# j4n1k/rl4co-slap

Measured on AMD Instinct MI355X. Metric: env-steps/sec (batch×decode) SLAP & TSP-100 at 1/2/4/8 MI355X, higher is better.
Workload: dtype u8+i64+f32

## Files before the change

rl4co_slap_amd/csrc/nearest.hip:

```cpp
#include "co_common.hpp"

using namespace co;

namespace {

constexpr int kNoNode = 0x7fffffff;

#ifndef CO_NEAREST_LDS_G
#define CO_NEAREST_LDS_G 4
#endif
#ifndef CO_NEAREST_CVRP_G
#define CO_NEAREST_CVRP_G 8
#endif

__global__ __launch_bounds__(256) void cvrp_pad_kernel(int64_t B, const int32_t* __restrict__ len,
                                                       const int32_t* __restrict__ tmax,
                                                       int64_t* __restrict__ acts_out,
                                                       int64_t* __restrict__ cur_out,
                                                       float* __restrict__ used_out) {
  const int T = *tmax;
  for (int64_t b = (int64_t)blockIdx.x * blockDim.x + threadIdx.x; b < B;
       b += (int64_t)gridDim.x * blockDim.x) {
    const int L = len[b];
    for (int t = L; t < T; ++t) acts_out[(int64_t)t * B + b] = 0;
    if (L < T) {
      cur_out[b] = 0;
      used_out[b] = 0.f;
    }
  }
}

typedef float v2f __attribute__((ext_vector_type(2)));

constexpr int clog2(int v) {
  int b = 0;
  while ((1 << b) < v) ++b;
  return b;
}

__device__ __forceinline__ uint32_t med3u(uint32_t a, uint32_t b, uint32_t c) {
  uint32_t r;
  asm("v_med3_u32 %0, %1, %2, %3" : "=v"(r) : "v"(a), "v"(b), "v"(c));
  return r;
}

template <int G, int EPL>
__device__ __forceinline__ void lds_load_x(const float* __restrict__ rowx, int sl,
                                           v2f (&x2)[EPL / 2]) {
  const float* r = rowx + sl;
#pragma unroll
  for (int p = 0; p < EPL / 2; ++p) x2[p] = (v2f){r[2 * p * G], r[(2 * p + 1) * G]};
}

template <int G, int EPL, bool DEM>
__device__ __forceinline__ void lds_scan(const v2f (&x2)[EPL / 2], float cx, float cy,
                                         const v2f (&y2)[EPL / 2], const v2f (&dm2)[EPL / 2],
                                         float used, float vcap, uint32_t& m1, uint32_t& m2) {
  constexpr uint32_t BM = (1u << clog2(G * EPL)) - 1u;
  const v2f cx2 = {cx, cx}, cy2 = {cy, cy};
  const v2f u2 = {used, used};
  uint32_t a1 = 0xffffffffu, a2 = 0xffffffffu, b1 = 0xffffffffu, b2 = 0xffffffffu;
#pragma unroll
  for (int p = 0; p < EPL / 2; ++p) {
    const v2f dx = x2[p] - cx2, dy = y2[p] - cy2;
    const v2f s = dx * dx + dy * dy;
    v2f du = {0.f, 0.f};
    if (DEM) du = dm2[p] + u2;
#pragma unroll
    for (int h = 0; h < 2; ++h) {
      uint32_t key = (__float_as_uint(s[h]) & ~BM) | (uint32_t)((2 * p + h) * G);
      if (DEM && du[h] > vcap) key = 0xffffffffu;
      if (p & 1) {
        b2 = med3u(b1, b2, key);
        b1 = min(b1, key);
      } else {
        a2 = med3u(a1, a2, key);
        a1 = min(a1, key);
      }
    }
  }
  m1 = min(a1, b1);
  m2 = med3u(a1, b1, min(a2, b2));
}

template <int G>
__device__ __forceinline__ void grp_min2(uint32_t& m1, uint32_t& m2) {
#define CO_MIN2(C)                                             \
  {                                                            \
    const uint32_t t1 = dpp_u<C>(m1), t2 = dpp_u<C>(m2);       \
    m2 = med3u(m1, t1, min(m2, t2));                           \
    m1 = min(m1, t1);                                          \
  }
  if (G >= 2) CO_MIN2(0xB1);
  if (G >= 4) CO_MIN2(0x4E);
  if (G >= 8) CO_MIN2(0x141);
  if (G >= 16) CO_MIN2(0x140);
#undef CO_MIN2
  if (G >= 32) {
    const auto a = __builtin_amdgcn_permlane16_swap(m1, m1, false, false);
    const auto b = __builtin_amdgcn_permlane16_swap(m2, m2, false, false);
    m2 = med3u(a[0], a[1], min(b[0], b[1]));
    m1 = min(a[0], a[1]);
  }
  if (G >= 64) {
    const auto a = __builtin_amdgcn_permlane32_swap(m1, m1, false, false);
    const auto b = __builtin_amdgcn_permlane32_swap(m2, m2, false, false);
    m2 = med3u(a[0], a[1], min(b[0], b[1]));
    m1 = min(a[0], a[1]);
  }
}

template <int G, int EPL, bool DEM>
__device__ __noinline__ int lds_exact(const float* __restrict__ rowx,
                                      const float2* __restrict__ lrow,
                                      const float* __restrict__ drow, int lo, int hi, int sl,
                                      float cx, float cy, float used, float vcap) {
  float best = __builtin_inff();
  int bi = kNoNode;
#pragma unroll 2
  for (int k = 0; k < EPL; ++k) {
    const int c = k * G + sl;
    const int ci = c < lo ? 0 : (c > hi ? hi - lo : c - lo);
    const float d = edge_len(cx, cy, rowx[c], lrow[ci].y);
    const bool fits = !DEM || !(drow[ci] + used > vcap);
    if (fits && d < best) {
      best = d;
      bi = c;
    }
  }
  grp_argmin_split<G>(best, bi);
  return bi;
}

template <int G, int EPL, bool DEM>
__device__ __forceinline__ int lds_nearest(const float* __restrict__ rowx,
                                           const v2f (&x2)[EPL / 2], int sl, float cx, float cy,
                                           const v2f (&y2)[EPL / 2], const v2f (&dm2)[EPL / 2],
                                           float used, float vcap,
                                           const float2* __restrict__ lrow,
                                           const float* __restrict__ drow, int lo, int hi) {
  constexpr uint32_t BM = (1u << clog2(G * EPL)) - 1u;
  constexpr float kWin = 1.0f + (float)(1u << clog2(G * EPL)) * 0x1p-20f;
  uint32_t m1, m2;
  lds_scan<G, EPL, DEM>(x2, cx, cy, y2, dm2, used, vcap, m1, m2);
  m1 |= (uint32_t)sl;
  m2 |= (uint32_t)sl;
  grp_min2<G>(m1, m2);
  const uint32_t t1 = m1 & ~BM, t2 = m2 & ~BM;
  const bool none = t1 >= 0x7fc00000u;
  const bool ok = none | ((t1 - 0x0d800000u < 0x7f800000u - 0x0d800000u) &
                          (t2 > __float_as_uint(__uint_as_float(t1) * kWin)));
  int w = none ? kNoNode : (int)(m1 & BM);
  if (__builtin_expect(__any(!ok), 0))
    w = lds_exact<G, EPL, DEM>(rowx, lrow, drow, lo, hi, sl, cx, cy, used, vcap);
  return w;
}

template <int G>
struct TermAcc {
  double sum = 0.0;
  float hold = 0.f;
  __device__ __forceinline__ void add(float sq, int t, int sl) {
    const int r = t & (G - 1);
    hold = sl == r ? sq : hold;
    if (r == G - 1) {
      asm volatile("");
      sum += (double)__builtin_sqrtf(hold);
      hold = 0.f;
    }
  }
  __device__ __forceinline__ double total() {
    return grp_sum_f64<G>(sum + (double)__builtin_sqrtf(hold));
  }
};

template <int G, int EPL>
__global__ __launch_bounds__(64) void tsp_nearest_lds_kernel(
    int64_t B, int N, const float2* __restrict__ locs, int64_t* __restrict__ acts_out,
    uint8_t* __restrict__ mask_out, int64_t* __restrict__ first_out,
    int64_t* __restrict__ cur_out, int64_t* __restrict__ i_out, uint8_t* __restrict__ done_out,
    uint8_t* __restrict__ step_reward_out, float* __restrict__ reward_out) {
  static_assert(EPL % 2 == 0 && (G & (G - 1)) == 0 && G * EPL <= 1024, "slot pairs");
  constexpr int IPW = 64 / G, SLOTS = G * EPL;
  __shared__ float2 s_x[IPW * SLOTS / 2];
  const int lane = threadIdx.x, sl = lane % G, gi = lane / G, gbase = lane - sl;
  const int64_t base = (int64_t)blockIdx.x * IPW;
  if (base >= B) return;
  const int64_t b = base + gi;
  const bool valid = b < B;
  const int64_t bb = valid ? b : B - 1;
  const float2* lrow = locs + bb * N;
  float* const rowx = reinterpret_cast<float*>(s_x) + gi * SLOTS;
  const float qnan = __builtin_nanf("");
  v2f y2[EPL / 2];
#pragma unroll
  for (int k = 0; k < EPL; ++k) {
    const int c = k * G + sl;
    const float2 q = lrow[c < N ? c : N - 1];
    rowx[c] = c < N ? q.x : qnan;
    y2[k >> 1][k & 1] = c < N ? q.y : 0.f;
  }
  const v2f nodem[EPL / 2] = {};
  const float2 q0 = lrow[0];
  __syncthreads();
  rowx[0] = qnan;
  float cx = q0.x, cy = q0.y;
  if (valid && sl == 0) acts_out[bb] = 0;
  TermAcc<G> len;
  int cur = 0;
  v2f x2[EPL / 2];
  lds_load_x<G, EPL>(rowx, sl, x2);
  for (int t = 1; t < N; ++t) {
    int a = lds_nearest<G, EPL, false>(rowx, x2, sl, cx, cy, y2, nodem, 0.f, 0.f, lrow,
                                       nullptr, 0, N - 1);
    a = a == kNoNode ? 0 : a;
    float* px = rowx + a;
    const float2 wq = lrow[a];
    const float wx = wq.x, wy = wq.y;
    *px = qnan;
    lds_load_x<G, EPL>(rowx, sl, x2);
    const float dx = wx - cx, dy = wy - cy;
    len.add(dx * dx + dy * dy, t, sl);
    cx = wx;
    cy = wy;
    cur = a;
    if (valid && sl == 0) acts_out[(int64_t)t * B + bb] = a;
  }
  const float ex = q0.x - cx, ey = q0.y - cy;
  len.add(ex * ex + ey * ey, N, sl);
  const double tour = len.total();
  if (!valid) return;
  uint8_t* mrow = mask_out + bb * N;
  for (int c = sl; c < N; c += G) mrow[c] = 0;
  if (sl == 0) {
    first_out[bb] = 0;
    cur_out[bb] = cur;
    i_out[bb] = N;
    done_out[bb] = 1;
    step_reward_out[bb] = 0;
    reward_out[bb] = -(float)tour;
  }
}

template <int G, int EPL>
__global__ __launch_bounds__(64) void cvrp_nearest_lds_kernel(
    int64_t B, int N, const float2* __restrict__ depot, const float2* __restrict__ locs_in,
    const float* __restrict__ demand, float vcap, int max_steps, int64_t* __restrict__ acts_out,
    float2* __restrict__ locs_out, int64_t* __restrict__ cur_out, float* __restrict__ used_out,
    float* __restrict__ vcap_out, uint8_t* __restrict__ visited_out,
    uint8_t* __restrict__ mask_out, uint8_t* __restrict__ done_out,
    uint8_t* __restrict__ step_reward_out, float* __restrict__ reward_out,
    int32_t* __restrict__ len_out, int32_t* __restrict__ tmax, int32_t* status) {
  static_assert(EPL % 2 == 0 && (G & (G - 1)) == 0 && G * EPL <= 1024, "slot pairs");
  constexpr int IPW = 64 / G, SLOTS = G * EPL;
  __shared__ float2 s_x[IPW * SLOTS / 2];
  const int lane = threadIdx.x, sl = lane % G, gi = lane / G, gbase = lane - sl;
  const int M = N + 1;
  const int64_t base = (int64_t)blockIdx.x * IPW;
  if (base >= B) return;
  const int64_t b = base + gi;
  const bool valid = b < B;
  const int64_t bb = valid ? b : B - 1;
  const float2* lrow = locs_in + bb * N;
  const float* drow = demand + bb * N;
  float* const rowx = reinterpret_cast<float*>(s_x) + gi * SLOTS;
  const float qnan = __builtin_nanf("");
  const float2 dep = depot[bb];
  v2f y2[EPL / 2], dm2[EPL / 2];
#pragma unroll
  for (int k = 0; k < EPL; ++k) {
    const int c = k * G + sl;
    const int ci = c < 1 ? 0 : (c <= N ? c - 1 : N - 1);
    const float2 lq = lrow[ci];
    const float ld = drow[ci];
    const float2 q = c == 0 ? dep : (c <= N ? lq : make_float2(qnan, 0.f));
    const float d = (c >= 1 && c <= N) ? ld : 0.f;
    if (valid && locs_out && c <= N) locs_out[bb * M + c] = q;
    rowx[c] = c == 0 ? qnan : q.x;
    y2[k >> 1][k & 1] = q.y;
    dm2[k >> 1][k & 1] = d;
  }
  __syncthreads();
  float cx = dep.x, cy = dep.y, used = 0.f;
  uint32_t st = 0;
  int cur = 0;
  bool done = false;
  TermAcc<G> dist;
  v2f x2[EPL / 2];
  lds_load_x<G, EPL>(rowx, sl, x2);
  int t = 0;
  for (; t < max_steps; ++t) {
    if (__ballot(!done) == 0) break;
    const int w = lds_nearest<G, EPL, true>(rowx, x2, sl, cx, cy, y2, dm2, used, vcap, lrow,
                                            drow, 1, N);
    const int a = w == kNoNode ? 0 : w;
    float* px = rowx + a;
    const int ai = a == 0 ? 0 : a - 1;
    const float2 wq = lrow[ai];
    const float wx = wq.x, wy = wq.y, wd = drow[ai];
    if (!done && a != 0) *px = qnan;
    lds_load_x<G, EPL>(rowx, sl, x2);
    const float2 q = a == 0 ? dep : make_float2(wx, wy);
    const float dx = q.x - cx, dy = q.y - cy;
    dist.add(done ? 0.f : dx * dx + dy * dy, t, sl);
    if (done) continue;
    used = a != 0 ? (used + wd) * 1.0f : 0.0f;
    st = ((st & 0x8000ffffu) + (a != 0 ? 1u : 0u)) | ((uint32_t)(t + 1) << 16) |
         (a == 0 ? 0x80000000u : 0u);
    cur = a;
    cx = q.x;
    cy = q.y;
    if (valid && sl == 0) acts_out[(int64_t)t * B + bb] = a;
    done = (st & 0x8000ffffu) == (0x80000000u | (uint32_t)N);
  }
  const int len = (int)((st >> 16) & 0x7fffu);
  const float ex = dep.x - cx, ey = dep.y - cy;
  dist.add(ex * ex + ey * ey, t, sl);
  const double tour = dist.total();
  bool any_feas = false;
  uint8_t* vrow = visited_out + bb * M;
  uint8_t* mrow = mask_out + bb * M;
#pragma unroll
  for (int k = 0; k < EPL; ++k) {
    const int c = k * G + sl;
    const bool v = c == 0 ? (st >> 31) != 0 : __builtin_isnan(rowx[c]);
    const bool feas = c >= 1 && c <= N && !v && !(dm2[k >> 1][k & 1] + used > vcap);
    any_feas |= feas;
    if (valid && c <= N) {
      vrow[c] = v;
      if (c >= 1) mrow[c] = feas;
    }
  }
  const uint64_t gmask = (G == 64 ? ~0ull : ((1ull << G) - 1ull)) << gbase;
  const bool anyf = (__ballot(any_feas) & gmask) != 0;
  if (valid && sl == 0) {
    mrow[0] = !((cur == 0) && anyf);
    cur_out[bb] = cur;
    used_out[bb] = used;
    vcap_out[bb] = vcap;
    done_out[bb] = done;
    step_reward_out[bb] = 0;
    reward_out[bb] = -(float)tour;
    len_out[bb] = len;
    if (!done) set_status(status, CO_ST_TRUNCATED);
    atomicMax(tmax, len);
  }
}

inline unsigned lds_grid(int64_t B, int G) {
  return cover_grid(B, 64 / G, 64);
}

}

int co_internal_tsp_nearest_rollout(int64_t B, int64_t N, const float* locs, int64_t* acts_out,
                                    uint8_t* mask_out, int64_t* first_out, int64_t* cur_out,
                                    int64_t* i_out, uint8_t* done_out, uint8_t* step_reward_out,
                                    float* reward_out, void* stream) {
  const float2* l2 = reinterpret_cast<const float2*>(locs);
  hipStream_t s = (hipStream_t)stream;
  if (lds_grid(B, 4) == 0) return CO_E_INVAL;
#define CO_TSPL(G, EPL)                                                                        \
  hipLaunchKernelGGL((tsp_nearest_lds_kernel<G, EPL>), dim3(lds_grid(B, G)), dim3(64), 0, s, B,  \
                     (int)N, l2, acts_out, mask_out, first_out, cur_out, i_out, done_out,        \
                     step_reward_out, reward_out)
  if (N <= 32) CO_TSPL(4, 8);
  else if (N <= 64) CO_TSPL(4, 16);
  else if (N <= 104 && CO_NEAREST_LDS_G == 4) CO_TSPL(4, 26);
  else if (N <= 112) CO_TSPL(8, 14);
  else if (N <= 128) CO_TSPL(8, 16);
  else if (N <= 256) CO_TSPL(8, 32);
  else if (N <= 512) CO_TSPL(16, 32);
  else CO_TSPL(32, 32);
#undef CO_TSPL
  return launch_status();
}

extern "C" int co_cvrp_rollout(int64_t B, int64_t N, const float* depot, const float* locs,
                               const float* demand, float vcap, int64_t max_steps,
                               int64_t* acts_out, float* locs_out, int64_t* cur_out,
                               float* used_out, float* vcap_out, uint8_t* visited_out,
                               uint8_t* mask_out, uint8_t* done_out, uint8_t* step_reward_out,
                               float* reward_out, int32_t* len_out, int32_t* steps_out,
                               int32_t* status, void* stream) {
  if (B < 0 || B > 0x7fffffff || N <= 0 || N > 1023 || max_steps <= 0 || max_steps > 0x7fff)
    return CO_E_INVAL;
  if (B == 0) return CO_OK;
  if (!depot || !locs || !demand || !acts_out || !cur_out || !used_out || !vcap_out ||
      !visited_out || !mask_out || !done_out || !step_reward_out || !reward_out || !len_out ||
      !steps_out || !status)
    return CO_E_INVAL;
  if ((reinterpret_cast<uintptr_t>(depot) | reinterpret_cast<uintptr_t>(locs) |
       reinterpret_cast<uintptr_t>(locs_out)) & 7)
    return CO_E_ALIGN;
  hipStream_t s = (hipStream_t)stream;
  if (lds_grid(B, 4) == 0) return CO_E_INVAL;
  if (zero_i32(steps_out, s) != hipSuccess) return launch_status();
  const float2* d2 = reinterpret_cast<const float2*>(depot);
  const float2* l2 = reinterpret_cast<const float2*>(locs);
  float2* lo = reinterpret_cast<float2*>(locs_out);
  const int64_t M = N + 1;
#define CO_CVRPL(G, EPL)                                                                       \
  hipLaunchKernelGGL((cvrp_nearest_lds_kernel<G, EPL>), dim3(lds_grid(B, G)), dim3(64), 0, s, B, \
                     (int)N, d2, l2, demand, vcap, (int)max_steps, acts_out, lo, cur_out,        \
                     used_out, vcap_out, visited_out, mask_out, done_out, step_reward_out,       \
                     reward_out, len_out, steps_out, status)
  if (M <= 32) CO_CVRPL(4, 8);
  else if (M <= 64) CO_CVRPL(4, 16);
  else if (M <= 112) CO_CVRPL(CO_NEAREST_CVRP_G, 112 / CO_NEAREST_CVRP_G);
  else if (M <= 128) CO_CVRPL(8, 16);
  else if (M <= 256) CO_CVRPL(8, 32);
  else if (M <= 512) CO_CVRPL(16, 32);
  else CO_CVRPL(32, 32);
#undef CO_CVRPL
  hipLaunchKernelGGL(cvrp_pad_kernel, dim3(grid_for(B, 256, 2048)), dim3(256), 0, s, B, len_out,
                     steps_out, acts_out, cur_out, used_out);
  return launch_status();
}
```

Measured before the change: 353.9 billion.

## Compact unvisited TSP nodes into shrinking LDS slots during greedy decode

Restructures the greedy nearest-neighbour TSP decode into phases. As nodes are visited, the remaining live nodes are compacted into fewer per-lane slots with an index table stored in LDS, so each step's scan covers only the remaining candidates instead of all N. A packed min2 key with a tolerance window selects the winner, falling back to an exact scan when the gap between the two best candidates is ambiguous. It also raises the launch-bounds occupancy hint. The cost is added compaction passes with barriers, extra code paths and register pressure.

```diff
diff --git a/rl4co_slap_amd/csrc/nearest.hip b/rl4co_slap_amd/csrc/nearest.hip
--- a/rl4co_slap_amd/csrc/nearest.hip
+++ b/rl4co_slap_amd/csrc/nearest.hip
@@ -174,14 +174,168 @@
   }
 };
 
+constexpr int even_up(int v) { return (v + 1) & ~1; }
+
+constexpr int tsp_next_epl(int epl0, int idx_bytes, int epl) {
+  if (epl <= 2) return 0;
+  int n = even_up(epl >= 12 ? (2 * epl + 2) / 3 : (epl + 1) / 2);
+  const int room = (epl0 * 4 / (4 + idx_bytes)) & ~1;
+  if (epl == epl0 && n > room) n = room;
+  return n;
+}
+
+template <int G, class IdxT>
+__device__ __noinline__ int tsp_exact(const float* __restrict__ rowx, const IdxT* tab,
+                                      const float2* __restrict__ lrow, int N, int epl, int sl,
+                                      float cx, float cy) {
+  float best = __builtin_inff();
+  int bi = kNoNode;
+#pragma unroll 2
+  for (int k = 0; k < epl; ++k) {
+    const int p = k * G + sl;
+    int c = tab ? (int)tab[p] : p;
+    c = c < N ? c : N - 1;
+    const float d = edge_len(cx, cy, rowx[p], lrow[c].y);
+    if (d < best) {
+      best = d;
+      bi = p;
+    }
+  }
+  grp_argmin_split<G>(best, bi);
+  return bi;
+}
+
+template <int G, class IdxT>
+struct TspRun {
+  int64_t B, bb;
+  int N, sl, gbase, t, cur;
+  bool valid;
+  const float2* __restrict__ lrow;
+  float* rowx;
+  IdxT* tab;
+  int64_t* __restrict__ acts_out;
+  float cx, cy;
+  TermAcc<G> len;
+};
+
+template <int G, bool TAB, class IdxT>
+__device__ __forceinline__ void tsp_visit(TspRun<G, IdxT>& r, int w) {
+  const bool hit = w != kNoNode;
+  const int p = hit ? w : 0;
+  int a = p;
+  if (TAB) {
+    const int c = (int)r.tab[p];
+    a = hit ? c : 0;
+  }
+  const float2 wq = r.lrow[a];
+  const float wx = wq.x, wy = wq.y;
+  if (!TAB || hit) r.rowx[p] = __builtin_nanf("");
+  const float dx = wx - r.cx, dy = wy - r.cy;
+  r.len.add(dx * dx + dy * dy, r.t, r.sl);
+  r.cx = wx;
+  r.cy = wy;
+  r.cur = a;
+  if (r.valid && r.sl == 0) r.acts_out[(int64_t)r.t * r.B + r.bb] = a;
+}
+
+template <int G, int EPL, bool TAB, class IdxT>
+__device__ __forceinline__ void tsp_step(TspRun<G, IdxT>& r, v2f (&x2)[EPL / 2],
+                                         const v2f (&y2)[EPL / 2]) {
+  constexpr uint32_t BM = (1u << clog2(G * EPL)) - 1u;
+  constexpr float kWin = 1.0f + (float)(1u << clog2(G * EPL)) * 0x1p-20f;
+  const v2f nodem[EPL / 2] = {};
+  uint32_t m1, m2;
+  lds_scan<G, EPL, false>(x2, r.cx, r.cy, y2, nodem, 0.f, 0.f, m1, m2);
+  m1 |= (uint32_t)r.sl;
+  m2 |= (uint32_t)r.sl;
+  grp_min2<G>(m1, m2);
+  const uint32_t t1 = m1 & ~BM, t2 = m2 & ~BM;
+  const bool none = t1 >= 0x7fc00000u;
+  const bool ok = none | ((t1 - 0x0d800000u < 0x7f800000u - 0x0d800000u) &
+                          (t2 > __float_as_uint(__uint_as_float(t1) * kWin)));
+  int w = none ? kNoNode : (int)(m1 & BM);
+  if (__builtin_expect(__any(!ok), 0))
+    w = tsp_exact<G, IdxT>(r.rowx, TAB ? r.tab : nullptr, r.lrow, r.N, EPL, r.sl, r.cx, r.cy);
+  tsp_visit<G, TAB, IdxT>(r, w);
+  lds_load_x<G, EPL>(r.rowx, r.sl, x2);
+}
+
+template <int G, int EPL, int NEXT, bool TAB, class IdxT>
+__device__ __forceinline__ bool tsp_compact(const TspRun<G, IdxT>& r, const v2f (&x2)[EPL / 2],
+                                            v2f (&nx2)[NEXT / 2], v2f (&ny2)[NEXT / 2]) {
+  static_assert(G <= 32, "a group's ballot bits fit 32 bits");
+  const uint32_t gm = G == 32 ? 0xffffffffu : (1u << G) - 1u, lm = (1u << r.sl) - 1u;
+  uint32_t live = 0;
+#pragma unroll
+  for (int k = 0; k < EPL; ++k) live += x2[k >> 1][k & 1] == x2[k >> 1][k & 1] ? 1u : 0u;
+  live = grp_reduce<G>(live, [](uint32_t a, uint32_t b) { return a + b; });
+  if (__any(live > (uint32_t)(G * NEXT))) return false;
+  int node[TAB ? EPL : 1];
+  if (TAB) {
+#pragma unroll
+    for (int k = 0; k < EPL; ++k) node[k] = (int)r.tab[k * G + r.sl];
+  }
+  __syncthreads();
+  uint32_t run = 0;
+#pragma unroll
+  for (int k = 0; k < EPL; ++k) {
+    const float x = x2[k >> 1][k & 1];
+    const uint32_t bits = (uint32_t)(__ballot(x == x) >> r.gbase) & gm;
+    const uint32_t pos = run + __popc(bits & lm);
+    run += __popc(bits);
+    if (x == x) {
+      r.rowx[pos] = x;
+      r.tab[pos] = (IdxT)(TAB ? node[k] : k * G + r.sl);
+    }
+  }
+#pragma unroll
+  for (int k = 0; k < NEXT; ++k)
+    if ((uint32_t)(k * G + r.sl) >= run) r.rowx[k * G + r.sl] = __builtin_nanf("");
+  __syncthreads();
+  lds_load_x<G, NEXT>(r.rowx, r.sl, nx2);
+  const float* lf = reinterpret_cast<const float*>(r.lrow);
+#pragma unroll
+  for (int k = 0; k < NEXT; ++k) {
+    const int p = k * G + r.sl;
+    const bool in = (uint32_t)p < run;
+    const int c = in ? (int)r.tab[p] : 0;
+    const float y = lf[2 * c + 1];
+    ny2[k >> 1][k & 1] = in ? y : 0.f;
+  }
+  return true;
+}
+
+template <int G, int EPL0, int EPL, class IdxT>
+__device__ __forceinline__ void tsp_phases(TspRun<G, IdxT>& r, v2f (&x2)[EPL / 2],
+                                           const v2f (&y2)[EPL / 2]) {
+  constexpr int NEXT = tsp_next_epl(EPL0, (int)sizeof(IdxT), EPL);
+  constexpr bool TAB = EPL != EPL0;
+  const int stop = NEXT ? r.N - G * NEXT : r.N;
+  for (; r.t < stop; ++r.t) tsp_step<G, EPL, TAB, IdxT>(r, x2, y2);
+  if constexpr (NEXT != 0) {
+    if (r.t >= r.N) return;
+    v2f nx2[NEXT / 2], ny2[NEXT / 2];
+    if (tsp_compact<G, EPL, NEXT, TAB, IdxT>(r, x2, nx2, ny2)) {
+      tsp_phases<G, EPL0, NEXT, IdxT>(r, nx2, ny2);
+      return;
+    }
+    for (; r.t < r.N; ++r.t)
+      tsp_visit<G, TAB, IdxT>(r, tsp_exact<G, IdxT>(r.rowx, TAB ? r.tab : nullptr, r.lrow, r.N,
+                                                    EPL, r.sl, r.cx, r.cy));
+  }
+}
+
 template <int G, int EPL>
-__global__ __launch_bounds__(64) void tsp_nearest_lds_kernel(
+__global__ __launch_bounds__(64, EPL <= 26 ? 4 : 3) void tsp_nearest_lds_kernel(
     int64_t B, int N, const float2* __restrict__ locs, int64_t* __restrict__ acts_out,
     uint8_t* __restrict__ mask_out, int64_t* __restrict__ first_out,
     int64_t* __restrict__ cur_out, int64_t* __restrict__ i_out, uint8_t* __restrict__ done_out,
     uint8_t* __restrict__ step_reward_out, float* __restrict__ reward_out) {
   static_assert(EPL % 2 == 0 && (G & (G - 1)) == 0 && G * EPL <= 1024, "slot pairs");
   constexpr int IPW = 64 / G, SLOTS = G * EPL;
+  using IdxT = std::conditional_t<SLOTS <= 256, uint8_t, uint16_t>;
+  constexpr int EPL1 = tsp_next_epl(EPL, (int)sizeof(IdxT), EPL);
+  static_assert(EPL1 * (4 + (int)sizeof(IdxT)) <= EPL * 4, "the index table fits the row");
   __shared__ float2 s_x[IPW * SLOTS / 2];
   const int lane = threadIdx.x, sl = lane % G, gi = lane / G, gbase = lane - sl;
   const int64_t base = (int64_t)blockIdx.x * IPW;
@@ -200,32 +354,19 @@
     rowx[c] = c < N ? q.x : qnan;
     y2[k >> 1][k & 1] = c < N ? q.y : 0.f;
   }
-  const v2f nodem[EPL / 2] = {};
   const float2 q0 = lrow[0];
   __syncthreads();
   rowx[0] = qnan;
-  float cx = q0.x, cy = q0.y;
   if (valid && sl == 0) acts_out[bb] = 0;
-  TermAcc<G> len;
-  int cur = 0;
   v2f x2[EPL / 2];
   lds_load_x<G, EPL>(rowx, sl, x2);
-  for (int t = 1; t < N; ++t) {
-    int a = lds_nearest<G, EPL, false>(rowx, x2, sl, cx, cy, y2, nodem, 0.f, 0.f, lrow,
-                                       nullptr, 0, N - 1);
-    a = a == kNoNode ? 0 : a;
-    float* px = rowx + a;
-    const float2 wq = lrow[a];
-    const float wx = wq.x, wy = wq.y;
-    *px = qnan;
-    lds_load_x<G, EPL>(rowx, sl, x2);
-    const float dx = wx - cx, dy = wy - cy;
-    len.add(dx * dx + dy * dy, t, sl);
-    cx = wx;
-    cy = wy;
-    cur = a;
-    if (valid && sl == 0) acts_out[(int64_t)t * B + bb] = a;
-  }
+  TspRun<G, IdxT> run = {B,    bb,   N,    sl,   gbase, 1,    0,
+                         valid, lrow, rowx, reinterpret_cast<IdxT*>(rowx + G * EPL1),
+                         acts_out, q0.x, q0.y, TermAcc<G>()};
+  tsp_phases<G, EPL, EPL, IdxT>(run, x2, y2);
+  const float cx = run.cx, cy = run.cy;
+  const int cur = run.cur;
+  TermAcc<G> len = run.len;
   const float ex = q0.x - cx, ey = q0.y - cy;
   len.add(ex * ex + ey * ey, N, sl);
   const double tour = len.total();
```

Result: no change. 353.1 billion (-0.2%).
